# M4THYOU/TokenDagger

Measured on AMD Instinct MI355X. Metric: GB/s raw text tokenized (Llama-4 vocab, 1024 MB corpus), higher is better.
Workload: dtype u8

## Files before the change

### tokendagger_amd/csrc/td_kernels.hip

```cpp
#include <hip/hip_runtime.h>
#include <stdlib.h>

#include "td_kernels.h"

namespace td {

#ifdef TD_ABLATE
#define TD_STOP(n) (a.stop_after == (n))
#else
#define TD_STOP(n) false
#endif

struct LdsSrc {
    const uint8_t* txt;
    const uint32_t* docw;
    int64_t lo, hi;
    __device__ __forceinline__ uint32_t byte(int64_t i) const { return txt[i]; }
    __device__ __forceinline__ bool doc(int64_t i) const { return (docw[i >> 5] >> (i & 31)) & 1u; }
};
struct GlobSrc {
    const uint8_t* text;
    const uint32_t* docbits;
    int64_t lo, hi;
    __device__ __forceinline__ uint32_t byte(int64_t i) const { return text[i]; }
// ... 582 lines not shown
static_assert(SLAB_MIDS >= FZ_NPC + 8, "a slab holds the slots of the fullest tile the fused loop takes");
constexpr int FZ_R_BYTES = ((FZ_R_SPLIT_END > FZ_R_TOK_END ? FZ_R_SPLIT_END : FZ_R_TOK_END) + 15) & ~15;
constexpr int PD_KIND = 0;
constexpr int PD_TILE = 1, PD_NP = 2, PD_N0 = 3, PD_COUNT = 4, PD_NMISS = 5, PD_FDD = 6, PD_EXT0 = 7;
constexpr int PD_WORDS = 8;
static_assert(SLAB_MAX_MISSES == 2 * K_MISS_LISTED_MAX, "slab layout");
#ifndef TD_LB_MAX_POLLS
#define TD_LB_MAX_POLLS 2
#endif
#ifndef TD_LB_DRAIN_POLLS
#define TD_LB_DRAIN_POLLS 64
#endif
#ifndef TD_LB_MAX_ROUNDS
#define TD_LB_MAX_ROUNDS 4
#endif
#ifndef TD_FUSED_MIN_WAVES
#define TD_FUSED_MIN_WAVES 7
#endif

#ifndef TD_DIRECT_MIN_WAVES
#define TD_DIRECT_MIN_WAVES 6
#endif
static_assert(TD_FUSED_MIN_WAVES < 7 || FZ_R_BYTES <= 11072, "seven workgroups per CU: 22 752 B of LDS each, of which s_R may have 11 072");
template <uint32_t PV, bool FUSED, bool DIRECT>
__global__ __launch_bounds__(K_THREADS, !FUSED ? TD_SPLIT_MIN_WAVES : DIRECT ? TD_DIRECT_MIN_WAVES : TD_FUSED_MIN_WAVES) void td_split_tiles(const EncodeArgs a_kern) {
    static_assert(FUSED || !DIRECT, "direct placement is part of the fused tile loop");
    __shared__ __attribute__((aligned(16))) uint8_t s_txt[K_WIN];
    __shared__ __attribute__((aligned(16))) uint8_t s_R[FZ_R_BYTES];
    uint32_t* const s_cm = reinterpret_cast<uint32_t*>(s_R);
    uint16_t* const s_heads = reinterpret_cast<uint16_t*>(s_R + FZ_R_HEADS);
    uint16_t* const s_cold = reinterpret_cast<uint16_t*>(s_R + FZ_R_COLD);
    __shared__ uint32_t s_start[K_WIN / 32 + 3];
    __shared__ uint32_t s_doc[K_WIN / 32 + 2];
    __shared__ uint8_t s_lut[128];
    __shared__ uint8_t s_fcls[16];
    __shared__ uint32_t s_nh, s_cur, s_ncold, s_nonascii;
    __shared__ int s_last;
    __shared__ int s_cross;
    __shared__ uint32_t s_defer;
    __shared__ int s_next[2];

    const int tid = threadIdx.x;
#ifdef TD_FUSED_TIMING
    unsigned long long tt[16] = {0, 0, 0, 0, 0, 0, 0, 0, 0, 0, 0, 0, 0, 0, 0, 0}, t_last = __builtin_readcyclecounter(), t_total0 = t_last, n_tiles_done = 0;
#define FZ_TICK(i) { const unsigned long long t_now = __builtin_readcyclecounter(); tt[i] += t_now - t_last; t_last = t_now; FZ_FRESH }
#else
#define FZ_TICK(i) FZ_FRESH
#endif
#ifndef TD_ARGS_IN_REGISTERS
    (void)a_kern;
    FreshArgs a{kernarg_args()};
    FreshTables T{(const __attribute__((address_space(4))) Tables*)a->Tp};
#define FZ_FRESH { a.refresh(); T.refresh(); }
#else
    const KeptArgs a{&a_kern};
    const Tables T_kept = uniform_tables(a->Tp);
    const KeptTables T{&T_kept};
#define FZ_FRESH
#endif
    for (int q = tid; q < 128; q += K_THREADS) s_lut[q] = (uint8_t)feature_of_class(T->ascii_cls[q]);
    if (tid < 16) s_fcls[tid] = (uint8_t)feature_of_class((uint32_t)tid);
    if (tid == 0) s_nonascii = 0;
    if (tid < 2) s_doc[K_WIN / 32 + tid] = 0;
    static_assert(K_WIN / 32 + 2 == CM_STRIDE, "the document bits cover the words the stored masks have");
    __shared__ __attribute__((aligned(16))) uint32_t s_kmask[FUSED ? (P12_MAXLEN + 1) * 4 : 4];
    __shared__ uint32_t s_wave[8];
    __shared__ uint32_t s_hflags[2], s_nrec[2], s_ncoldp;
    __shared__ uint32_t s_rec[2][K_MISS_LISTED_MAX];
    __shared__ unsigned long long s_pend[48];
    __shared__ uint32_t s_npend;
// ... 25 lines not shown
        if (tid < (int)(P12_MAXLEN + 1) * 4) {
            const int len = tid >> 2, w = tid & 3, nb = len - 4 * w;
            s_kmask[tid] = w == 3 || nb <= 0 ? 0u : nb >= 4 ? 0xFFFFFFFFu : (1u << (8 * nb)) - 1u;
        }
        if (tid == 0) { s_nflagl = 0; s_npend = 0; s_brk = 0; }
        if (DIRECT && tid < SLAB_RING * PD_WORDS) (&s_pd[0][0])[tid] = 0;
        if (tid < 2) s_stat[tid] = 0;
    }
    __syncthreads();

#ifndef TD_FUSED_NPRE
#define TD_FUSED_NPRE 0
#endif
    constexpr int NPF = (K_WIN / 16 + K_THREADS - 1) / K_THREADS;
    constexpr int NPRE = FUSED ? TD_FUSED_NPRE : NPF;
    uint4 pf[NPF];
    const int64_t nwords = (a->n + 31) >> 5;
    auto interior = [&](int64_t w0) { return a->text_aligned && w0 >= 0 && w0 + K_WIN <= a->n; };
    uint32_t pfd0 = 0, pfd1 = 0, pffd0 = 0xFFFFFFFFu, pffd1 = 0xFFFFFFFFu;
#ifdef TD_TEXT_L2_PREFETCH
    uint32_t pft = 0;
#endif
    static_assert(K_WIN / 32 <= 2 * K_THREADS, "two prefetched document words per lane cover the window");
    auto load_window = [&](int64_t w0) {
        {
            const int64_t gw0 = (w0 >> 5) + tid, gw1 = gw0 + K_THREADS;
            pfd0 = (gw0 >= 0 && gw0 < nwords) ? a->docbits[gw0] : 0u;
            pfd1 = (tid < K_WIN / 32 - K_THREADS && gw1 >= 0 && gw1 < nwords) ? a->docbits[gw1] : 0u;
            if (FUSED) {
                const int64_t t4 = (w0 + K_HL) / K_TILE;
                pffd0 = t4 < a->n_tiles ? a->tile_first_doc[t4] : 0xFFFFFFFFu;
                pffd1 = t4 + 1 < a->n_tiles ? a->tile_first_doc[t4 + 1] : 0xFFFFFFFFu;
            }
        }
        if (!interior(w0)) return;
#ifdef TD_TEXT_L2_PREFETCH
        if (FUSED && NPRE == 0 && tid < (K_WIN + 63) / 64) pft = *reinterpret_cast<const volatile uint8_t*>(a->text + w0 + 64 * tid);
#endif
        const uint4* src16 = reinterpret_cast<const uint4*>(a->text + w0);
#pragma unroll
        for (int q = 0; q < NPRE; ++q)
            if (q < NPF - 1 || tid < K_WIN / 16 - (NPF - 1) * K_THREADS) pf[q] = nt_load16(src16 + q * K_THREADS + tid);
    };
#pragma unroll
    for (int q = 0; q < NPF; ++q) pf[q] = make_uint4(0, 0, 0, 0);
    int first_tile = (int)blockIdx.x;
    if constexpr (DIRECT) {
        if (tid == 0) s_next[0] = (int)atomicAdd(a->tile_draw, 1u);
        __syncthreads();
        first_tile = __builtin_amdgcn_readfirstlane(s_next[0]);
        __syncthreads();
    }
    if (first_tile < a->n_stiles) load_window((int64_t)first_tile * KS_TILE - K_HL);
    const int tid_outer = tid;
#ifndef TD_FUSED_STATIC_TILES
    constexpr bool DRAW = FUSED;
#else
    constexpr bool DRAW = false;
#endif
    int next_tile = 0, par = 0;
    int ring = 0;
    if (DRAW && !DIRECT && tid == 0) s_next[0] = (int)(blockIdx.x + gridDim.x);
    for (int tile = first_tile;; tile = DRAW ? next_tile : tile + (int)gridDim.x) {
        const bool have = tile < a->n_stiles;
        if (!have) {
            bool pending = false;
            if constexpr (DIRECT)
                for (int r = 0; r < SLAB_RING; ++r) pending = pending || s_pd[r][PD_KIND] != 0u;
            if (!pending) break;
        }
        int tid_opaque = tid_outer;
        asm volatile("" : "+v"(tid_opaque));
        const int tid = tid_opaque, lane = tid & 63;
        const int64_t tile_g0 = (int64_t)tile * KS_TILE;
        const int64_t wg0 = tile_g0 - K_HL;
        const int tile_hi = K_HL + (int)((a->n - tile_g0 < KS_TILE) ? (a->n - tile_g0) : KS_TILE);
// ... 9 lines not shown
        const uint32_t* const pslab = a->slab + ((size_t)blockIdx.x * SLAB_RING + ring) * SLAB_WORDS;
        if (DIRECT && pkind) {
            B = (int)s_pd[ring][PD_TILE];
            pnp = s_pd[ring][PD_NP]; pn0 = s_pd[ring][PD_N0]; pcount = s_pd[ring][PD_COUNT]; pnm = s_pd[ring][PD_NMISS]; pext0 = s_pd[ring][PD_EXT0];
            const uint32_t nv4 = (pnp + 3u) >> 2;
#pragma unroll
            for (int q = 0; q < 3; ++q) {
                xs[q] = make_uint4(0, 0, 0, 0);
                if ((uint32_t)tid + 256u * q < nv4) xs[q] = reinterpret_cast<const uint4*>(pslab)[tid + 256 * q];
            }
            const uint32_t pfdd = s_pd[ring][PD_FDD];
            pdm = (int64_t)pfdd + tid;
            pdpos = a->n;
            if (pkind == 1u && pfdd != 0xFFFFFFFFu && pdm < a->n_docs) { pdpos = a->doc_offsets[pdm]; pdsl = a->doc_slot[pdm]; }
            const int idx0 = B - 1 - tid;
            stw = (pkind == 1u && idx0 >= 0) ? __hip_atomic_load(&a->tile_state[idx0], __ATOMIC_RELAXED, __HIP_MEMORY_SCOPE_AGENT) : (TS_PREFIX << 62);
        }
        if (have) {
#ifdef TD_TEXT_L2_PREFETCH
        if (FUSED) asm volatile("" :: "v"(pft));
#endif

        uint32_t hib = 0;
        if (interior(wg0)) {
#pragma unroll
            for (int q = NPRE; q < NPF; ++q)
                if (q < NPF - 1 || tid < K_WIN / 16 - (NPF - 1) * K_THREADS) pf[q] = nt_load16(reinterpret_cast<const uint4*>(a->text + wg0) + q * K_THREADS + tid);
#pragma unroll
            for (int q = 0; q < NPF; ++q)
                if (q < NPF - 1 || tid < K_WIN / 16 - (NPF - 1) * K_THREADS) {
                    reinterpret_cast<uint4*>(s_txt)[q * K_THREADS + tid] = pf[q];
                    hib |= pf[q].x | pf[q].y | pf[q].z | pf[q].w;
                }
        } else {
            hib = stage_window_edge(s_txt, a->text, a->n, wg0, tid, K_WIN / 16);
        }
#pragma unroll
        for (int q = 0; q < 2; ++q) {
            const int w = tid + q * K_THREADS;
            if (w < K_WIN / 32) {
                uint32_t dw = q ? pfd1 : pfd0;
                const int64_t g = wg0 + (int64_t)w * 32;
                if (g + 32 > a->n) dw |= (g >= a->n) ? 0xFFFFFFFFu : ~((1u << (int)(a->n - g)) - 1u);
                s_doc[w] = dw;
            }
        }
        if (DRAW && DIRECT && tid == 0) s_next[0] = (int)atomicAdd(a->tile_draw, 1u);
        if (!FUSED && tile + (int)gridDim.x < a->n_stiles) load_window(wg0 + (int64_t)gridDim.x * KS_TILE);
        for (int w = tid; w < K_WIN / 32 + 3; w += K_THREADS) s_start[w] = 0;
        if (tid == 0) { s_nh = 0; s_cur = 0; s_ncold = 0; s_last = -1; s_cross = -1; s_defer = 0; }
        if (__ballot((hib & 0x80808080u) != 0) && lane == 0) s_nonascii = 1;
        }
        auto lb_post = [&](unsigned long long w) {
            const uint32_t status = (uint32_t)(w >> 62);
            const uint64_t na = __ballot(status != (uint32_t)TS_AGG);
            const int first = na ? (int)td_ctz64(na) : 64;
            const uint32_t mysum = wave_incl_scan(lane < first ? (uint32_t)w : 0u, lane);
            if (lane == 63) { s_lbs[tid >> 6][0] = (uint32_t)first; s_lbs[tid >> 6][1] = mysum; }
            if (lane == first) { s_lbs[tid >> 6][2] = status; s_lbv[tid >> 6] = w & TS_VALUE_MASK; }
        };
        if (DIRECT && pkind == 1u) lb_post(stw);
        __syncthreads();
        if (DIRECT && pkind) {
            const uint32_t* const slab = pslab;
            const uint32_t* const meta = slab + SLAB_META;
            const int64_t pg0 = (int64_t)B * KS_TILE, pg1 = (pg0 + KS_TILE < a->n) ? pg0 + KS_TILE : a->n;
            long long base = -1;
            if (pkind == 1u) {
                long long acc = 0;
                int j = B - 1, polls = 0, rounds = 0;
                for (;;) {
                    uint32_t tstatus = (uint32_t)TS_AGG;
                    unsigned long long tval = 0;
                    int tdist = 0;
#pragma unroll
                    for (int w = 0; w < K_THREADS / 64; ++w) {
                        if (tstatus == (uint32_t)TS_AGG) {
                            acc += s_lbs[w][1];
                            const int f = (int)s_lbs[w][0];
                            if (f < 64) { tstatus = s_lbs[w][2]; tval = s_lbv[w]; tdist = w * 64 + f; }
                        }
                    }
                    if (tstatus == (uint32_t)TS_PREFIX) { base = acc + (long long)tval; break; }
                    if (tstatus == (uint32_t)TS_BROKEN) { base = -1; break; }
                    if (tstatus == (uint32_t)TS_NONE) {
                        if (++polls > (have ? TD_LB_MAX_POLLS : TD_LB_DRAIN_POLLS)) { base = -2; break; }
                        j -= tdist;
                        __builtin_amdgcn_s_sleep(8);
                    } else {
                        if (++rounds >= TD_LB_MAX_ROUNDS) { base = -2; break; }
                        j -= K_THREADS;
                    }
                    __syncthreads();
                    const int idx = j - tid;
                    lb_post(idx >= 0 ? __hip_atomic_load(&a->tile_state[idx], __ATOMIC_RELAXED, __HIP_MEMORY_SCOPE_AGENT) : (TS_PREFIX << 62));
                    __syncthreads();
                }
            }
            FZ_TICK(8)
            const int tB4 = B * (KS_TILE / K_TILE);
            const bool ptwo = tB4 + 1 < a->n_tiles;
            uint32_t* const st0 = a->stage + (size_t)tB4 * K_STAGE;
            auto shift_of = [&](uint32_t k, int& mine) { return fz_shift_of(meta, pnm, k, &mine); };
            if (pkind == 1u && base >= 0) {
                int32_t* const dst = a->out_tokens + base;
                const bool fits = base + (long long)pcount <= (long long)a->out_cap;
                if (fits && pnm == 0u) {
#pragma unroll
                    for (int q = 0; q < 3; ++q) {
                        const uint32_t v = (uint32_t)tid + 256u * q;
                        if (4u * v + 4u <= pnp) {
                            u32x4a4 o;
                            o.x = xs[q].x; o.y = xs[q].y; o.z = xs[q].z; o.w = xs[q].w;
                            TD_NT_STORE(o, reinterpret_cast<u32x4a4*>(dst + 4u * v));
                        } else if (4u * v < pnp) {
                            dst[4u * v] = (int32_t)xs[q].x;
                            if (4u * v + 1u < pnp) dst[4u * v + 1u] = (int32_t)xs[q].y;
                            if (4u * v + 2u < pnp) dst[4u * v + 2u] = (int32_t)xs[q].z;
                        }
// ... 46 lines not shown
                    fz_stage_with_misses(slab, st0, a->merge_out + (size_t)tB4 * K_STAGE, pnp, pn0, pnm);
                }
                if (pkind == 1u && tid == 0) {
                    uint32_t m0 = 0, m1 = 0;
                    for (uint32_t q = 0; q < pnm; ++q) { if (meta[SLAB_MAX_MISSES + q] >> 12) m1 = 1; else m0 = 1; }
                    a->tile_count[tB4] = pn0 | (m0 ? TILE_MISS_LISTED : 0u);
                    a->tile_extra[tB4] = pext0;
                    if (ptwo) {
                        a->tile_count[tB4 + 1] = (pnp - pn0) | (m1 ? TILE_MISS_LISTED : 0u);
                        a->tile_extra[tB4 + 1] = pcount - pnp - pext0;
                    }
                    if (base == -1) {
                        __hip_atomic_store(&a->tile_state[B], TS_BROKEN << 62, __ATOMIC_RELAXED, __HIP_MEMORY_SCOPE_AGENT);
                        s_brk = 1u;
                    } else {
                        s_stat[1] += 1u;
                    }
                }
            }
            if (tid == 0) s_pd[ring][PD_KIND] = 0;
            FZ_TICK(11)
        }
        if (!have) {
            __syncthreads();
            ring = __builtin_amdgcn_readfirstlane(ring + 1 == SLAB_RING ? 0 : ring + 1);
            continue;
        }
        {
        FZ_TICK(0)
        const bool tile_ascii = !s_nonascii;

        LdsSrc src;
        src.txt = s_txt;
        src.docw = s_doc;
        src.lo = (wg0 < 0) ? -wg0 : 0;
        src.hi = (a->n - wg0 < K_WIN) ? (a->n - wg0) : K_WIN;
        if (tid < 2 * CM_COUNT) s_cm[(tid >> 1) * CM_STRIDE + 2 * K_MWORDS + (tid & 1)] = 0;
        auto emit_masks = [&](int it, uint32_t flo, uint32_t fhi, uint32_t pf) {
            const uint64_t P = transpose8x8(((uint64_t)fhi << 32) | flo);
            const uint32_t plo = (uint32_t)P, phi = (uint32_t)(P >> 32);
            const uint32_t mU = plo & 0xFF, mW = (plo >> 8) & 0xFF, mX = (plo >> 16) & 0xFF, mS = plo >> 24;
            const uint32_t nraw = phi & 0xFF, mCR = (phi >> 8) & 0xFF, mSL = (phi >> 16) & 0xFF, mC = phi >> 24;
            const uint32_t mN = nraw & ~mX & ~mS, mA = nraw & mX;
            const uint32_t mD = reinterpret_cast<const uint8_t*>(s_doc)[it];
            const uint32_t mSY = sync_byte(mU, mW, mX, mS, mN, mCR, mSL, mC, mD, mA, pf, PV);
            static_assert(CM_U == 0 && CM_W == 1 && CM_X == 2 && CM_S == 3 && CM_NRAW == 4 && CM_CR == 5 && CM_TR == 6 &&
                          CM_C == 7 && CM_SYNC == 8, "stored mask order");
            uint8_t* o = reinterpret_cast<uint8_t*>(s_cm) + it;
            constexpr int MB = CM_STRIDE * 4;
            o[0 * MB] = (uint8_t)mU; o[1 * MB] = (uint8_t)mW; o[2 * MB] = (uint8_t)mX; o[3 * MB] = (uint8_t)mS;
            o[4 * MB] = (uint8_t)nraw; o[5 * MB] = (uint8_t)mCR; o[6 * MB] = (uint8_t)(mCR | mSL); o[7 * MB] = (uint8_t)mC;
            o[8 * MB] = (uint8_t)mSY;
        };
        constexpr int P1_ITEMS = K_WIN / 8;
        if (tile_ascii) {
            for (int it = tid; it < P1_ITEMS; it += K_THREADS) {
                const uint2 t8 = reinterpret_cast<const uint2*>(s_txt)[it];
                const uint32_t flo = (uint32_t)s_lut[t8.x & 0x7F] | ((uint32_t)s_lut[(t8.x >> 8) & 0x7F] << 8) |
                                     ((uint32_t)s_lut[(t8.x >> 16) & 0x7F] << 16) | ((uint32_t)s_lut[t8.x >> 24] << 24);
                const uint32_t fhi = (uint32_t)s_lut[t8.y & 0x7F] | ((uint32_t)s_lut[(t8.y >> 8) & 0x7F] << 8) |
                                     ((uint32_t)s_lut[(t8.y >> 16) & 0x7F] << 16) | ((uint32_t)s_lut[t8.y >> 24] << 24);
                uint32_t pf = __shfl_up(fhi >> 24, 1);
                if (lane == 0) pf = it > 0 ? (uint32_t)s_lut[s_txt[it * 8 - 1]] : 0u;
                emit_masks(it, flo, fhi, pf);
            }
        } else {
        constexpr int P1_WAVES = K_THREADS / 64, P1_PER_WAVE = (P1_ITEMS / P1_WAVES) & ~63;
        static_assert(P1_ITEMS - P1_WAVES * P1_PER_WAVE <= 64, "the items left over are one more pass of the last wavefront");
        uint32_t carry_st = 0x100u, carry_pf = 0;
        const int n_pass = P1_PER_WAVE / 64 + ((tid >> 6) == P1_WAVES - 1 ? 1 : 0);
        const uint8_t* const t_ascii = T->ascii_cls;
        const uint16_t* const t_u1 = T->ucls1;
        const uint8_t* const t_u2 = T->ucls2;
        for (int q = 0; q < n_pass; ++q) {
            const int it = (tid >> 6) * P1_PER_WAVE + q * 64 + lane;
            if (it >= P1_ITEMS) break;
            const uint2 t8 = reinterpret_cast<const uint2*>(s_txt)[it];
            uint32_t flo, fhi;
            uint32_t st_out = 0;
// ... 100 lines not shown
                carry_st = (uint32_t)__builtin_amdgcn_readlane((int)st_out, 63);
                if (lead_conts) {
                    const bool known = !(st_in & 0x100u);
                    const int claim = (int)(st_in >> 9);
                    for (int k = 0; k < lead_conts; ++k) {
                        const uint32_t f = (known && k < claim) ? ((st_in & 0xFFu) | FB_C) : feature_at_v(t_ascii, t_u1, t_u2, s_txt, s_doc, (int)src.lo, (int)src.hi, it * 8 + k);
                        if (k < 4) flo |= f << (8 * k); else fhi |= f << (8 * (k - 4));
                    }
                }
            }
            uint32_t pf = __shfl_up(fhi >> 24, 1);
            if (lane == 0 && q > 0) pf = carry_pf;
            carry_pf = (uint32_t)__builtin_amdgcn_readlane((int)(fhi >> 24), 63);
            if (lane == 0 && q == 0) {
                pf = 0;
                if (it > 0) {
                    const uint32_t pb = s_txt[it * 8 - 1];
                    pf = (pb < 0x80) ? (uint32_t)s_lut[pb] : feature_at_v(t_ascii, t_u1, t_u2, s_txt, s_doc, (int)src.lo, (int)src.hi, it * 8 - 1);
                }
            }
            emit_masks(it, flo, fhi, pf);
        }
        }
        __syncthreads();
        FZ_TICK(1)
        if (tid == 0) s_nonascii = 0;
        if (TD_STOP(12)) continue;

        {
            constexpr bool FAST = !(PV & (PV_GPT2 | PV_LEADING_CONTRACTION | PV_PLAIN_LETTERS | PV_WS_EOS_FIRST));
            auto load_view64 = [&](BitWin& v, int j) {
                uint64_t s[CM_COUNT];
#pragma unroll
                for (int k = 0; k < CM_COUNT; ++k) s[k] = ((uint64_t)s_cm[k * CM_STRIDE + j + 1] << 32) | s_cm[k * CM_STRIDE + j];
                cm_expand(v, s, ((uint64_t)s_doc[j + 1] << 32) | s_doc[j]);
            };
            auto load_view32 = [&](BitWin32& v, int j, uint32_t sh) {
                uint32_t s[CM_COUNT];
#pragma unroll
                for (int k = 0; k < CM_COUNT; ++k) s[k] = __funnelshift_r(s_cm[k * CM_STRIDE + j], s_cm[k * CM_STRIDE + j + 1], sh);
                cm_expand(v, s, __funnelshift_r(s_doc[j], s_doc[j + 1], sh));
            };
            auto defer = [&](int64_t g) {
                if (FUSED) s_defer = 1;
                const uint32_t q = atomicAdd(a->slow_count, 1u);
                if (q < a->slow_cap) a->slow_list[q] = g;
                else raise(a, TD_E_SCRATCH, g);
// ... 29 lines not shown
                    un = (uint32_t)split_unresolved_heads(wv, PV, &extra) & sy;
                    extra &= (uint64_t)sy << 3;
                    extra &= room >= 64 ? ~0ull : room <= 0 ? 0ull : ((1ull << room) - 1ull);
                    st0 |= (uint32_t)extra;
                    extra_hi = (uint32_t)(extra >> 32);
                } else {
                    un = (uint32_t)split_unresolved_heads(wv, PV) & sy;
                }
                s_start[b0 >> 5] = st0;
                if (sy) atomicMax(&s_last, b0 + 31 - (int)__clz(sy));
                const uint32_t cnt = __popc(un);
                const uint32_t incl = wave_incl_scan(cnt, lane);
                uint32_t base = 0;
                if (lane == 63 && incl) base = atomicAdd(&s_nh, incl);
                base = (uint32_t)__builtin_amdgcn_readlane((int)base, 63);
                uint32_t idx = base + incl - cnt;
                while (un) {
                    const int bit = __ffs(un) - 1;
                    un &= un - 1u;
                    if (idx < (uint32_t)KS_HCAP) s_heads[idx] = (uint16_t)(b0 + bit); else mine |= 1u << bit;
                    ++idx;
                }
            }
            __syncthreads();
            FZ_TICK(2)
            if (extra_hi) atomicOr(&s_start[(b0 >> 5) + 1], extra_hi);
            if (TD_STOP(13)) continue;
            {
                const uint32_t nh = s_nh < (uint32_t)KS_HCAP ? s_nh : (uint32_t)KS_HCAP;
                int p = -1;
                if (tid == 0) {
                    static_assert(K_HL % 64 == 0 && K_HL >= 64, "left halo = whole mask words");
                    const uint32_t* const sync32 = s_cm + CM_SYNC * CM_STRIDE;
                    if (!(sync32[K_HL / 32] & 1u)) {
                        int sp = -1;
                        for (int w = K_HL / 64 - 1; w >= 0 && sp < 0; --w) {
                            uint64_t m = ((uint64_t)sync32[2 * w + 1] << 32) | sync32[2 * w];
                            if (w == 0) m &= ~0xFull;
                            if (m) sp = w * 64 + td_top64(m) - 1;
                        }
                        if (sp < 0) { a->tile_flag[tile] = 1; atomicAdd(a->far_count, 1u); if (FUSED) s_defer = 1; }
                        else p = sp;
                    }
                }
                if (tid == 1 && s_last >= 0) p = s_last;
                bool more = true;
                for (;;) {
                    const uint64_t nb = __ballot(p < 0);
                    if (nb && more) {
                        uint32_t base = 0;
                        if (lane == __ffsll((unsigned long long)nb) - 1) base = atomicAdd(&s_cur, (uint32_t)__popcll(nb));
                        base = (uint32_t)__builtin_amdgcn_readlane((int)base, __ffsll((unsigned long long)nb) - 1);
                        more = base + (uint32_t)__popcll(nb) < nh;
                        if (p < 0) {
                            const uint32_t idx = base + __builtin_amdgcn_mbcnt_hi((uint32_t)(nb >> 32), __builtin_amdgcn_mbcnt_lo((uint32_t)nb, 0u));
                            if (idx < nh) p = s_heads[idx];
                        }
                    }
                    if (!__ballot(p >= 0)) break;
                    if (p >= 0) {
                        BitWin32 v;
                        load_view32(v, p >> 5, (uint32_t)(p & 31));
                        const int avail = (K_LIM - p < 32) ? (K_LIM - p) : 32;
                        auto bytes = [&](int q) { return (uint32_t)s_txt[p + q]; };
                        const int r = FAST ? scan_piece_fast32(v, avail, bytes, PV) : scan_piece_p(WinP32(v, avail), bytes, PV);
                        if (r < 0) {
                            const uint32_t ci = atomicAdd(&s_ncold, 1u);
                            if (ci < (uint32_t)KS_CCAP) s_cold[ci] = (uint16_t)p; else walk(p);
                            p = -1;
                        } else {
                            const int e = p + r;
                            bool stop = true;
                            if (e >= tile_hi) crossed(e);
                            else {
                                stop = (r < 32) ? ((v.m[MK_SYNC] >> r) & 1u) : sync_at(e);
                                if (!stop && e >= K_HL) mark(e);
                            }
                            p = stop ? -1 : e;
                        }
                    }
                }
            }
            __syncthreads();
            {
                const uint32_t nc = s_ncold < (uint32_t)KS_CCAP ? s_ncold : (uint32_t)KS_CCAP;
                for (uint32_t i = tid; i < nc; i += K_THREADS) walk(s_cold[i]);
                while (mine) {
                    const int bit = __ffs(mine) - 1;
                    mine &= mine - 1u;
                    walk(b0 + bit);
                }
            }
        }
        __syncthreads();
        FZ_TICK(3)
        if (tid < KS_TILE / 32) {
            const int64_t g = tile_g0 + (int64_t)tid * 32;
            if (g < a->n) {
                uint32_t v = s_start[K_HL / 32 + tid];
                if (g + 32 > a->n) v &= (1u << (int)(a->n - g)) - 1u;
                TD_NT_STORE(v, &a->startbits[(tile_g0 >> 5) + tid]);
            }
        }
        if constexpr (DRAW) {
            if constexpr (!DIRECT) {
                next_tile = __builtin_amdgcn_readfirstlane(s_next[par]);
                if (tid == 0) s_next[par ^ 1] = (int)(2u * gridDim.x + atomicAdd(a->tile_draw, 1u));
                par = __builtin_amdgcn_readfirstlane(par ^ 1);
            } else {
                next_tile = __builtin_amdgcn_readfirstlane(s_next[0]);
            }
            if (next_tile < a->n_stiles) load_window((int64_t)next_tile * KS_TILE - K_HL);
        } else if (FUSED && tile + (int)gridDim.x < a->n_stiles) {
            load_window(wg0 + (int64_t)gridDim.x * KS_TILE);
        }
        }
        if constexpr (FUSED) {
            constexpr int NT4 = KS_TILE / K_TILE;
            static_assert(NT4 == 2 && KS_CHUNK == 32, "two token tiles, a 32-bit START word per lane");
            const int cross = s_cross;
            const bool tile_deferred = s_defer != 0 || cross < 0;
            uint16_t* const s_plist = reinterpret_cast<uint16_t*>(s_R + FZ_R_PLIST);
            uint16_t* const s_coldk = reinterpret_cast<uint16_t*>(s_R + FZ_R_COLDK);
            uint16_t* const s_pb = reinterpret_cast<uint16_t*>(s_R + FZ_R_PB);
            const int wv = tid >> 6;
            const int tile4 = tile * NT4;
            const bool two = K_HL + K_TILE < tile_hi;
            const int b0 = K_HL + tid * KS_CHUNK;
            const uint32_t smask0 = s_start[b0 >> 5];
            const uint32_t cnt = __popc(smask0);
            const uint32_t incl = wave_incl_scan(cnt, lane);
            if (lane == 63) s_wave[wv] = incl;
            if (tid == 0) { s_hflags[0] = 0; s_hflags[1] = 0; s_nrec[0] = 0; s_nrec[1] = 0; s_ncoldp = 0; }
            __syncthreads();
            const uint32_t w0s = s_wave[0], w1s = s_wave[1], w2s = s_wave[2], w3s = s_wave[3];
            const uint32_t np = w0s + w1s + w2s + w3s, n0 = w0s + w1s;
            const uint32_t pbase = (wv > 0 ? w0s : 0u) + (wv > 1 ? w1s : 0u) + (wv > 2 ? w2s : 0u) + incl - cnt;
            const bool cand = DIRECT && !s_brk;
            auto break_chain = [&]() {
                __hip_atomic_store(&a->tile_state[tile], TS_BROKEN << 62, __ATOMIC_RELAXED, __HIP_MEMORY_SCOPE_AGENT);
                s_brk = 1u;
            };
            if (tile_deferred || np > (uint32_t)FZ_NPC) {
                if (tid == 0) {
                    const uint32_t at = atomicAdd(a->deferred_count, two ? 2u : 1u);
                    a->deferred_list[at] = (uint32_t)tile4;
                    if (two) a->deferred_list[at + 1] = (uint32_t)tile4 + 1u;
                    if (DIRECT) break_chain();
                }
            } else {
                {
                    uint32_t k = pbase, m = smask0;
                    while (m) {
                        const int b = __ffs(m) - 1;
                        m &= m - 1;
                        s_plist[k++] = (uint16_t)(b0 + b);
                    }
                }
                s_pb[tid] = (uint16_t)pbase;
                if (tid == 0) s_plist[np] = (uint16_t)cross;
                const uint64_t fdd = fd0 != 0xFFFFFFFFu ? fd0 : fd1;
                if (cand && tid == 0) { s_pd[ring][PD_FDD] = (uint32_t)fdd; s_pd[ring][PD_TILE] = (uint32_t)tile; s_pd[ring][PD_NP] = np; s_pd[ring][PD_N0] = n0; }
                const int64_t dmine = (int64_t)fdd + tid;
                const int64_t dpos = (fdd != 0xFFFFFFFFu && dmine < a->n_docs) ? a->doc_offsets[dmine] : a->n;
                __syncthreads();
                FZ_TICK(4)
                uint32_t* const slab = a->slab + ((size_t)blockIdx.x * SLAB_RING + ring) * SLAB_WORDS;
                uint32_t* const dst0 = cand ? slab : a->stage + (size_t)tile4 * K_STAGE;
                uint32_t* const dst1 = cand ? slab : dst0 + K_STAGE - n0;
                auto note_miss = [&](uint32_t k, uint32_t res) {
                    const uint32_t h = k >= n0 ? 1u : 0u;
                    const uint32_t mi = atomicAdd(&s_nrec[h], 1u);
                    if (mi < (uint32_t)K_MISS_LISTED_MAX) s_rec[h][mi] = ((k - (h ? n0 : 0u)) << 19) | (res & 0x7FFFFu);
                };
                auto miss_marker = [&](int i, uint32_t len) { return TOK_MISS | ((uint32_t)((i - K_HL) & (K_TILE - 1)) << 7) | len; };
                typedef uint32_t u32x4 __attribute__((ext_vector_type(4)));
                typedef const u32x4 __attribute__((address_space(1)))* gslot_t;
                gslot_t const p12 = (gslot_t)(uintptr_t)T->piece12_slots;
                const uint32_t p12_mask = T->piece12_mask;
                const bool fastpath = a->use_fastpath != 0;
                for (uint32_t kb = tid; kb < np; kb += K_THREADS * FZ_PB) {
                    u32x4 sl[FZ_PB];
                    uint32_t kk0[FZ_PB], kk1[FZ_PB], kk2[FZ_PB], il[FZ_PB];
#pragma unroll
                    for (int q = 0; q < FZ_PB; ++q) {
                        const uint32_t k = kb + (uint32_t)q * K_THREADS;
                        const bool on = k < np;
                        const int i = on ? s_plist[k] : K_HL;
                        const uint32_t len = on ? (uint32_t)s_plist[k + 1] - (uint32_t)i : 0u;
                        const uint32_t* wp = reinterpret_cast<const uint32_t*>(s_txt) + (i >> 2);
                        const uint32_t sh = (i & 3) * 8;
                        const uint32_t w0 = wp[0], w1 = wp[1], w2 = wp[2], w3 = wp[3];
                        const uint4 km = reinterpret_cast<const uint4*>(s_kmask)[len < P12_MAXLEN ? len : P12_MAXLEN];
                        kk0[q] = __funnelshift_r(w0, w1, sh) & km.x;
                        kk1[q] = __funnelshift_r(w1, w2, sh) & km.y;
                        kk2[q] = __funnelshift_r(w2, w3, sh) & km.z;
                        il[q] = ((uint32_t)i << 16) | (len < 0xFFFFu ? len : 0xFFFFu);
                        if (on) sl[q] = p12[hash_piece12(kk0[q], kk1[q], kk2[q], len) & p12_mask];
                    }
#pragma unroll
                    for (int q = 0; q < FZ_PB; ++q) {
                        const uint32_t k = kb + (uint32_t)q * K_THREADS;
                        if (k < np) {
                            const int i = (int)(il[q] >> 16);
                            const uint32_t len = il[q] & 0xFFFFu;
                            const u32x4 e = sl[q];
                            if (len <= P12_MAXLEN && fastpath &&
                                (e.w == 0u || (e.x == kk0[q] && e.y == kk1[q] && e.z == kk2[q] && (e.w >> 24) == (0x80u | len)))) {
                                const bool miss = e.w == 0u;
                                const uint32_t res = miss ? miss_marker(i, len) : (e.w & 0x1FFFFFu);
                                if (miss) {
                                    if (len == 1) raise(a, TD_E_UNKNOWN_BYTE, wg0 + i);
                                    note_miss(k, res);
                                }
                                (k < n0 ? dst0 : dst1)[k] = res;
                            } else {
                                const uint32_t j = atomicAdd(&s_ncoldp, 1u);
                                if (j < (uint32_t)FZ_CCAP) s_coldk[j] = (uint16_t)k;
                            }
                        }
                    }
                }
                __syncthreads();
                FZ_TICK(5)
                const uint32_t ncold = s_ncoldp;
                const bool cold_overflow = ncold > (uint32_t)FZ_CCAP;
                if (!cold_overflow) {
                    for (uint32_t c = tid; c < ncold; c += K_THREADS) {
                        const uint32_t k = s_coldk[c];
                        const int i = s_plist[k];
                        const uint32_t len = (uint32_t)s_plist[k + 1] - (uint32_t)i;
                        const uint32_t h = k >= n0 ? 1u : 0u;
                        uint32_t res = probe_piece_cold<true>(a, T, s_txt, T->byte_id, &s_hflags[h], wg0, i, len);
                        if ((res & 0xC0000000u) == TOK_MISS) { res = miss_marker(i, len); note_miss(k, res); }
                        (h ? dst1 : dst0)[k] = res;
                    }
                }
                __syncthreads();
                FZ_TICK(6)
                const bool resolved = cand && !cold_overflow && !(s_hflags[0] | s_hflags[1]) && s_nrec[0] <= (uint32_t)K_MISS_LISTED_MAX &&
                                      s_nrec[1] <= (uint32_t)K_MISS_LISTED_MAX;
                if (cold_overflow) {
                    if (tid == 0) {
                        const uint32_t at = atomicAdd(a->deferred_count, two ? 2u : 1u);
                        a->deferred_list[at] = (uint32_t)tile4;
                        if (two) a->deferred_list[at + 1] = (uint32_t)tile4 + 1u;
                        if (DIRECT) break_chain();
                    }
                } else if (resolved) {
                    FZ_TICK(12)
                    if (tid < 64) {
                        const uint32_t nr0 = s_nrec[0], nr1 = s_nrec[1], nm = nr0 + nr1;
                        uint32_t ext0 = 0, ext1 = 0;
                        if (nm) {
                            static_assert(2 * SLAB_MAX_MISSES * 4 * MG_UNIT * 4 <= FZ_R_COLDK, "keys + ids of the merged pieces fit the (dead) piece list");
                            uint32_t rec = 0, hh = 0;
                            if ((uint32_t)lane < nm) {
                                hh = (uint32_t)lane >= nr0 ? 1u : 0u;
                                rec = s_rec[hh][(uint32_t)lane - (hh ? nr0 : 0u)];
                            }
                            const uint32_t nt = fz_merge_piece(a->Tp, a->text, a->n, reinterpret_cast<uint32_t*>(s_R), slab, rec, hh, n0, tile_g0, a->err, a->err_pos);
                            const uint32_t e0 = wave_incl_scan((nt && !hh) ? nt - 1u : 0u, lane), e1 = wave_incl_scan((nt && hh) ? nt - 1u : 0u, lane);
                            ext0 = (uint32_t)__builtin_amdgcn_readlane((int)e0, 63);
                            ext1 = (uint32_t)__builtin_amdgcn_readlane((int)e1, 63);
                        }
                        FZ_TICK(13)
                        if (tid == 0) {
                            const uint32_t count = s_pd[ring][PD_NP] + ext0 + ext1;
                            s_pd[ring][PD_KIND] = 1u; s_pd[ring][PD_COUNT] = count; s_pd[ring][PD_NMISS] = nm; s_pd[ring][PD_EXT0] = ext0;
                            __hip_atomic_store(&a->tile_state[s_pd[ring][PD_TILE]], (TS_AGG << 62) | (unsigned long long)count, __ATOMIC_RELAXED, __HIP_MEMORY_SCOPE_AGENT);
                        }
                    }
                    FZ_TICK(7)
                    {
                        const int64_t tile_end_g = wg0 + tile_hi;
                        auto slot_of = [&](int64_t p) {
                            const int lp = (int)(p - tile_g0);
                            const uint32_t k = (uint32_t)s_pb[lp >> 5] + __popc(s_start[K_HL / 32 + (lp >> 5)] & ((1u << (lp & 31)) - 1u));
                            return k >= n0 ? k - n0 : k;
                        };
                        if (dpos < tile_end_g) {
                            a->doc_slot[dmine] = slot_of(dpos);
                            for (int64_t d = dmine + K_THREADS; d < a->n_docs; d += K_THREADS) {
                                const int64_t p = a->doc_offsets[d];
                                if (p >= tile_end_g) break;
                                a->doc_slot[d] = slot_of(p);
                            }
                        }
                    }
                    FZ_TICK(9)
                } else {
                if (DIRECT && tid == 0) {
                    break_chain();
                    if (cand) { s_pd[ring][PD_KIND] = 2u; s_pd[ring][PD_NMISS] = 0; }
                }
                if (tid < 64) {
#pragma unroll
                    for (uint32_t h = 0; h < 2; ++h) {
                        const uint32_t nr = s_nrec[h], np0 = s_npend;
                        const bool listed = nr && nr <= (uint32_t)K_MISS_LISTED_MAX;
                        if (listed && (uint32_t)tid < nr) s_pend[np0 + tid] = ((unsigned long long)((uint32_t)tile4 + h) << 32) | s_rec[h][tid];
                        const uint32_t np1 = listed ? np0 + nr : np0;
                        wave_sync_lds();
                        if (np1 > 48u - (uint32_t)K_MISS_LISTED_MAX) {
                            append_pending(np1);
                            wave_sync_lds();
                            if (tid == 0) s_npend = 0;
                        } else if (tid == 0) {
                            s_npend = np1;
                        }
                        wave_sync_lds();
                    }
                    if (tid == 0) {
#pragma unroll
                        for (uint32_t h = 0; h < 2; ++h) {
                            if (h == 1 && !two) break;
                            uint32_t fl = s_hflags[h];
                            const uint32_t nr = s_nrec[h];
                            if (nr > (uint32_t)K_MISS_LISTED_MAX) {
                                fl |= TILE_HAS_MISS;
                                uint32_t nf = s_nflagl;
                                s_flagl[nf++] = (uint32_t)tile4 + h;
                                if (nf == 32u) {
                                    const uint32_t at = atomicAdd(a->flagged_count, 32u);
                                    for (uint32_t q = 0; q < 32u; ++q) a->flagged_list[at + q] = s_flagl[q];
                                    nf = 0;
                                }
                                s_nflagl = nf;
                            } else if (nr) {
                                fl |= TILE_MISS_LISTED;
                            }
                            a->tile_count[tile4 + h] = (h ? np - n0 : n0) | fl;
                        }
                    }
                }
                FZ_TICK(7)
                {
                    const int64_t tile_end_g = wg0 + tile_hi;
                    auto slot_of = [&](int64_t p) {
                        const int lp = (int)(p - tile_g0);
                        const uint32_t k = (uint32_t)s_pb[lp >> 5] + __popc(s_start[K_HL / 32 + (lp >> 5)] & ((1u << (lp & 31)) - 1u));
                        return k >= n0 ? k - n0 : k;
                    };
                    if (dpos < tile_end_g) {
                        a->doc_slot[dmine] = slot_of(dpos);
                        for (int64_t d = dmine + K_THREADS; d < a->n_docs; d += K_THREADS) {
                            const int64_t p = a->doc_offsets[d];
                            if (p >= tile_end_g) break;
                            a->doc_slot[d] = slot_of(p);
                        }
                    }
                }
                FZ_TICK(9)
                }
            }
        }
        __syncthreads();
        ring = __builtin_amdgcn_readfirstlane(ring + 1 == SLAB_RING ? 0 : ring + 1);
        FZ_TICK(10)
#ifdef TD_FUSED_TIMING
        ++n_tiles_done;
#endif
    }
#ifdef TD_FUSED_TIMING
    if (FUSED && tid == 0 && (blockIdx.x % 211) == 0)
        printf("fused wg %d: %llu tiles, total %llu cycles | stage %llu masks %llu rules %llu heads %llu | list %llu probe %llu cold %llu bookkeeping %llu lookback %llu docs %llu tail %llu place %llu | t12 %llu t13 %llu\n",
               (int)blockIdx.x, n_tiles_done, (unsigned long long)(__builtin_readcyclecounter() - t_total0), tt[0], tt[1], tt[2], tt[3], tt[4], tt[5], tt[6], tt[7],
               tt[8], tt[9], tt[10], tt[11], tt[12], tt[13]);
#endif
    if constexpr (FUSED) {
        if (DIRECT && tid == 0 && s_stat[0]) atomicAdd(a->direct_tiles, s_stat[0]);
        if (DIRECT && tid == 0 && s_stat[1]) atomicAdd(a->direct_tiles + 1, s_stat[1]);
        if (tid < 64) append_pending(s_npend);
        if (tid == 0 && s_nflagl) {
            const uint32_t nf = s_nflagl, at = atomicAdd(a->flagged_count, nf);
            for (uint32_t q = 0; q < nf; ++q) a->flagged_list[at + q] = s_flagl[q];
        }
    }
}

struct WaveMaskP {
    const Tables& T;
    const uint8_t* text;
    const uint32_t* docbits;
    int64_t n, g;
    int o, lim;
    int lane;
    __device__ __forceinline__ uint32_t cf_at(int64_t pos) const {
        if (pos >= n) return F_DOC;
        GlobSrc src;
        src.text = text; src.docbits = docbits; src.lo = 0; src.hi = n;
// ... 3582 lines not shown
```

Before: 494.5.

## Rotate serial duties across wavefronts per tile to balance barrier waits

Introduces a duty roster that gives single-lane and single-wave duties (head seeding, bookkeeping, draw, zeroing, cold lookups, doc slots, the tail of the text staging) to different wavefronts, rotating by tile index. The aim is to stop wavefront 0 from always carrying the serial work so the other waves are not idle at each workgroup barrier. It also turns the document-word loads into unconditional clamped loads and adds barrier-wait timing instrumentation. The risk is extra index arithmetic and possible divergence in the lane remapping.

```diff
diff --git a/tokendagger_amd/csrc/td_kernels.hip b/tokendagger_amd/csrc/td_kernels.hip
--- a/tokendagger_amd/csrc/td_kernels.hip
+++ b/tokendagger_amd/csrc/td_kernels.hip
@@ -628,6 +628,29 @@
 #define TD_DIRECT_MIN_WAVES 6
 #endif
 static_assert(TD_FUSED_MIN_WAVES < 7 || FZ_R_BYTES <= 11072, "seven workgroups per CU: 22 752 B of LDS each, of which s_R may have 11 072");
+
+#ifndef TD_ROSTER
+#define TD_ROSTER 3
+#endif
+constexpr bool RS_STATIC = (TD_ROSTER & 1) != 0, RS_TURN = (TD_ROSTER & 2) != 0;
+constexpr int RS_STAGE = 2, RS_MASK = 0, RS_HEAD_LEFT = 1, RS_HEAD_LAST = 2, RS_WALK = 3, RS_DRAW = 0, RS_LOOKUP = 2, RS_COLD = 1,
+              RS_BOOK = 2, RS_DOCS = 3;
+static_assert(((RS_LOOKUP + 3) & 3) == RS_COLD, "the lookup loop's short wavefront owns the cold lookups");
+static_assert(RS_HEAD_LEFT != RS_MASK && RS_HEAD_LAST != RS_MASK && RS_HEAD_LEFT != RS_HEAD_LAST && RS_BOOK != RS_DOCS && RS_WALK != RS_HEAD_LAST &&
+              RS_COLD != RS_BOOK, "neighbouring duties have different owners");
+__device__ __forceinline__ int duty_owner(int duty, int tile) {
+    return ((RS_STATIC ? duty : 0) + (RS_TURN ? tile : 0)) & 3;
+}
+__device__ __forceinline__ int duty_lane(int tid, int duty, int tile) {
+    if constexpr (!RS_STATIC && !RS_TURN) return tid;
+    return (tid - 64 * duty_owner(duty, tile)) & (K_THREADS - 1);
+}
+__device__ __forceinline__ bool duty_wave(int tid, int duty, int tile) {
+    if constexpr (!RS_STATIC && !RS_TURN) return tid < 64;
+    return (tid >> 6) == duty_owner(duty, tile);
+}
+static_assert(K_THREADS == 256, "four wavefronts take turns");
+
 template <uint32_t PV, bool FUSED, bool DIRECT>
 __global__ __launch_bounds__(K_THREADS, !FUSED ? TD_SPLIT_MIN_WAVES : DIRECT ? TD_DIRECT_MIN_WAVES : TD_FUSED_MIN_WAVES) void td_split_tiles(const EncodeArgs a_kern) {
     static_assert(FUSED || !DIRECT, "direct placement is part of the fused tile loop");
@@ -650,8 +673,11 @@
 #ifdef TD_FUSED_TIMING
     unsigned long long tt[16] = {0, 0, 0, 0, 0, 0, 0, 0, 0, 0, 0, 0, 0, 0, 0, 0}, t_last = __builtin_readcyclecounter(), t_total0 = t_last, n_tiles_done = 0;
 #define FZ_TICK(i) { const unsigned long long t_now = __builtin_readcyclecounter(); tt[i] += t_now - t_last; t_last = t_now; FZ_FRESH }
+    unsigned long long tb[16] = {0, 0, 0, 0, 0, 0, 0, 0, 0, 0, 0, 0, 0, 0, 0, 0};
+#define FZ_SYNC(i) { const unsigned long long t_in = __builtin_readcyclecounter(); __syncthreads(); tb[i] += __builtin_readcyclecounter() - t_in; }
 #else
 #define FZ_TICK(i) FZ_FRESH
+#define FZ_SYNC(i) __syncthreads()
 #endif
 #ifndef TD_ARGS_IN_REGISTERS
     (void)a_kern;
@@ -723,11 +749,20 @@
     uint32_t pft = 0;
 #endif
     static_assert(K_WIN / 32 <= 2 * K_THREADS, "two prefetched document words per lane cover the window");
-    auto load_window = [&](int64_t w0) {
+    auto load_window = [&](int64_t w0, int wtile) {
+        const int rs = duty_lane(tid, RS_STAGE, wtile);
+        (void)rs;
         {
             const int64_t gw0 = (w0 >> 5) + tid, gw1 = gw0 + K_THREADS;
-            pfd0 = (gw0 >= 0 && gw0 < nwords) ? a->docbits[gw0] : 0u;
-            pfd1 = (tid < K_WIN / 32 - K_THREADS && gw1 >= 0 && gw1 < nwords) ? a->docbits[gw1] : 0u;
+            const bool in0 = gw0 >= 0 && gw0 < nwords, in1 = tid < K_WIN / 32 - K_THREADS && gw1 >= 0 && gw1 < nwords;
+            if constexpr (RS_STATIC || RS_TURN) {
+                const uint32_t d0 = a->docbits[in0 ? gw0 : 0], d1 = a->docbits[in1 ? gw1 : 0];
+                pfd0 = in0 ? d0 : 0u;
+                pfd1 = in1 ? d1 : 0u;
+            } else {
+                pfd0 = in0 ? a->docbits[gw0] : 0u;
+                pfd1 = in1 ? a->docbits[gw1] : 0u;
+            }
             if (FUSED) {
                 const int64_t t4 = (w0 + K_HL) / K_TILE;
                 pffd0 = t4 < a->n_tiles ? a->tile_first_doc[t4] : 0xFFFFFFFFu;
@@ -741,7 +776,7 @@
         const uint4* src16 = reinterpret_cast<const uint4*>(a->text + w0);
 #pragma unroll
         for (int q = 0; q < NPRE; ++q)
-            if (q < NPF - 1 || tid < K_WIN / 16 - (NPF - 1) * K_THREADS) pf[q] = nt_load16(src16 + q * K_THREADS + tid);
+            if (q < NPF - 1 || rs < K_WIN / 16 - (NPF - 1) * K_THREADS) pf[q] = nt_load16(src16 + q * K_THREADS + (q < NPF - 1 ? tid : rs));
     };
 #pragma unroll
     for (int q = 0; q < NPF; ++q) pf[q] = make_uint4(0, 0, 0, 0);
@@ -752,7 +787,7 @@
         first_tile = __builtin_amdgcn_readfirstlane(s_next[0]);
         __syncthreads();
     }
-    if (first_tile < a->n_stiles) load_window((int64_t)first_tile * KS_TILE - K_HL);
+    if (first_tile < a->n_stiles) load_window((int64_t)first_tile * KS_TILE - K_HL, first_tile);
     const int tid_outer = tid;
 #ifndef TD_FUSED_STATIC_TILES
     constexpr bool DRAW = FUSED;
@@ -808,14 +843,16 @@
 #endif
 
         uint32_t hib = 0;
+        const int rs = duty_lane(tid, RS_STAGE, tile);
         if (interior(wg0)) {
 #pragma unroll
             for (int q = NPRE; q < NPF; ++q)
-                if (q < NPF - 1 || tid < K_WIN / 16 - (NPF - 1) * K_THREADS) pf[q] = nt_load16(reinterpret_cast<const uint4*>(a->text + wg0) + q * K_THREADS + tid);
+                if (q < NPF - 1 || rs < K_WIN / 16 - (NPF - 1) * K_THREADS)
+                    pf[q] = nt_load16(reinterpret_cast<const uint4*>(a->text + wg0) + q * K_THREADS + (q < NPF - 1 ? tid : rs));
 #pragma unroll
             for (int q = 0; q < NPF; ++q)
-                if (q < NPF - 1 || tid < K_WIN / 16 - (NPF - 1) * K_THREADS) {
-                    reinterpret_cast<uint4*>(s_txt)[q * K_THREADS + tid] = pf[q];
+                if (q < NPF - 1 || rs < K_WIN / 16 - (NPF - 1) * K_THREADS) {
+                    reinterpret_cast<uint4*>(s_txt)[q * K_THREADS + (q < NPF - 1 ? tid : rs)] = pf[q];
                     hib |= pf[q].x | pf[q].y | pf[q].z | pf[q].w;
                 }
         } else {
@@ -832,9 +869,9 @@
             }
         }
         if (DRAW && DIRECT && tid == 0) s_next[0] = (int)atomicAdd(a->tile_draw, 1u);
-        if (!FUSED && tile + (int)gridDim.x < a->n_stiles) load_window(wg0 + (int64_t)gridDim.x * KS_TILE);
-        for (int w = tid; w < K_WIN / 32 + 3; w += K_THREADS) s_start[w] = 0;
-        if (tid == 0) { s_nh = 0; s_cur = 0; s_ncold = 0; s_last = -1; s_cross = -1; s_defer = 0; }
+        if (!FUSED && tile + (int)gridDim.x < a->n_stiles) load_window(wg0 + (int64_t)gridDim.x * KS_TILE, tile + (int)gridDim.x);
+        for (int w = rs; w < K_WIN / 32 + 3; w += K_THREADS) s_start[w] = 0;
+        if (rs == (RS_STATIC ? 64 : 0)) { s_nh = 0; s_cur = 0; s_ncold = 0; s_last = -1; s_cross = -1; s_defer = 0; }
         if (__ballot((hib & 0x80808080u) != 0) && lane == 0) s_nonascii = 1;
         }
         auto lb_post = [&](unsigned long long w) {
@@ -846,7 +883,7 @@
             if (lane == first) { s_lbs[tid >> 6][2] = status; s_lbv[tid >> 6] = w & TS_VALUE_MASK; }
         };
         if (DIRECT && pkind == 1u) lb_post(stw);
-        __syncthreads();
+        FZ_SYNC(0);
         if (DIRECT && pkind) {
             const uint32_t* const slab = pslab;
             const uint32_t* const meta = slab + SLAB_META;
@@ -877,10 +914,10 @@
                         if (++rounds >= TD_LB_MAX_ROUNDS) { base = -2; break; }
                         j -= K_THREADS;
                     }
-                    __syncthreads();
+                    FZ_SYNC(8);
                     const int idx = j - tid;
                     lb_post(idx >= 0 ? __hip_atomic_load(&a->tile_state[idx], __ATOMIC_RELAXED, __HIP_MEMORY_SCOPE_AGENT) : (TS_PREFIX << 62));
-                    __syncthreads();
+                    FZ_SYNC(8);
                 }
             }
             FZ_TICK(8)
@@ -973,7 +1010,7 @@
             FZ_TICK(11)
         }
         if (!have) {
-            __syncthreads();
+            FZ_SYNC(0);
             ring = __builtin_amdgcn_readfirstlane(ring + 1 == SLAB_RING ? 0 : ring + 1);
             continue;
         }
@@ -986,7 +1023,11 @@
         src.docw = s_doc;
         src.lo = (wg0 < 0) ? -wg0 : 0;
         src.hi = (a->n - wg0 < K_WIN) ? (a->n - wg0) : K_WIN;
-        if (tid < 2 * CM_COUNT) s_cm[(tid >> 1) * CM_STRIDE + 2 * K_MWORDS + (tid & 1)] = 0;
+        const int rm = duty_lane(tid, RS_MASK, tile);
+        {
+            const int rz = RS_STATIC ? (rm + 128) & (K_THREADS - 1) : rm;
+            if (rz < 2 * CM_COUNT) s_cm[(rz >> 1) * CM_STRIDE + 2 * K_MWORDS + (rz & 1)] = 0;
+        }
         auto emit_masks = [&](int it, uint32_t flo, uint32_t fhi, uint32_t pf) {
             const uint64_t P = transpose8x8(((uint64_t)fhi << 32) | flo);
             const uint32_t plo = (uint32_t)P, phi = (uint32_t)(P >> 32);
@@ -1005,7 +1046,7 @@
         };
         constexpr int P1_ITEMS = K_WIN / 8;
         if (tile_ascii) {
-            for (int it = tid; it < P1_ITEMS; it += K_THREADS) {
+            for (int it = rm; it < P1_ITEMS; it += K_THREADS) {
                 const uint2 t8 = reinterpret_cast<const uint2*>(s_txt)[it];
                 const uint32_t flo = (uint32_t)s_lut[t8.x & 0x7F] | ((uint32_t)s_lut[(t8.x >> 8) & 0x7F] << 8) |
                                      ((uint32_t)s_lut[(t8.x >> 16) & 0x7F] << 16) | ((uint32_t)s_lut[t8.x >> 24] << 24);
@@ -1152,7 +1193,7 @@
             emit_masks(it, flo, fhi, pf);
         }
         }
-        __syncthreads();
+        FZ_SYNC(1);
         FZ_TICK(1)
         if (tid == 0) s_nonascii = 0;
         if (TD_STOP(12)) continue;
@@ -1228,14 +1269,16 @@
                     ++idx;
                 }
             }
-            __syncthreads();
+            FZ_SYNC(2);
             FZ_TICK(2)
             if (extra_hi) atomicOr(&s_start[(b0 >> 5) + 1], extra_hi);
             if (TD_STOP(13)) continue;
             {
                 const uint32_t nh = s_nh < (uint32_t)KS_HCAP ? s_nh : (uint32_t)KS_HCAP;
                 int p = -1;
-                if (tid == 0) {
+                const int rh = duty_lane(tid, RS_HEAD_LEFT, tile);
+                constexpr int RH_LAST = RS_STATIC ? 64 * ((RS_HEAD_LAST - RS_HEAD_LEFT) & 3) : 1;
+                if (rh == 0) {
                     static_assert(K_HL % 64 == 0 && K_HL >= 64, "left halo = whole mask words");
                     const uint32_t* const sync32 = s_cm + CM_SYNC * CM_STRIDE;
                     if (!(sync32[K_HL / 32] & 1u)) {
@@ -1249,7 +1292,7 @@
                         else p = sp;
                     }
                 }
-                if (tid == 1 && s_last >= 0) p = s_last;
+                if (rh == RH_LAST && s_last >= 0) p = s_last;
                 bool more = true;
                 for (;;) {
                     const uint64_t nb = __ballot(p < 0);
@@ -1287,10 +1330,10 @@
                     }
                 }
             }
-            __syncthreads();
+            FZ_SYNC(14);
             {
                 const uint32_t nc = s_ncold < (uint32_t)KS_CCAP ? s_ncold : (uint32_t)KS_CCAP;
-                for (uint32_t i = tid; i < nc; i += K_THREADS) walk(s_cold[i]);
+                for (uint32_t i = (uint32_t)duty_lane(tid, RS_WALK, tile); i < nc; i += K_THREADS) walk(s_cold[i]);
                 while (mine) {
                     const int bit = __ffs(mine) - 1;
                     mine &= mine - 1u;
@@ -1298,7 +1341,7 @@
                 }
             }
         }
-        __syncthreads();
+        FZ_SYNC(3);
         FZ_TICK(3)
         if (tid < KS_TILE / 32) {
             const int64_t g = tile_g0 + (int64_t)tid * 32;
@@ -1311,14 +1354,14 @@
         if constexpr (DRAW) {
             if constexpr (!DIRECT) {
                 next_tile = __builtin_amdgcn_readfirstlane(s_next[par]);
-                if (tid == 0) s_next[par ^ 1] = (int)(2u * gridDim.x + atomicAdd(a->tile_draw, 1u));
+                if (duty_lane(tid, RS_DRAW, tile) == 0) s_next[par ^ 1] = (int)(2u * gridDim.x + atomicAdd(a->tile_draw, 1u));
                 par = __builtin_amdgcn_readfirstlane(par ^ 1);
             } else {
                 next_tile = __builtin_amdgcn_readfirstlane(s_next[0]);
             }
-            if (next_tile < a->n_stiles) load_window((int64_t)next_tile * KS_TILE - K_HL);
+            if (next_tile < a->n_stiles) load_window((int64_t)next_tile * KS_TILE - K_HL, next_tile);
         } else if (FUSED && tile + (int)gridDim.x < a->n_stiles) {
-            load_window(wg0 + (int64_t)gridDim.x * KS_TILE);
+            load_window(wg0 + (int64_t)gridDim.x * KS_TILE, tile + (int)gridDim.x);
         }
         }
         if constexpr (FUSED) {
@@ -1337,8 +1380,9 @@
             const uint32_t cnt = __popc(smask0);
             const uint32_t incl = wave_incl_scan(cnt, lane);
             if (lane == 63) s_wave[wv] = incl;
-            if (tid == 0) { s_hflags[0] = 0; s_hflags[1] = 0; s_nrec[0] = 0; s_nrec[1] = 0; s_ncoldp = 0; }
-            __syncthreads();
+            const int rd = duty_lane(tid, RS_DRAW, tile);
+            if (rd == (RS_STATIC ? 64 : 0)) { s_hflags[0] = 0; s_hflags[1] = 0; s_nrec[0] = 0; s_nrec[1] = 0; s_ncoldp = 0; }
+            FZ_SYNC(4);
             const uint32_t w0s = s_wave[0], w1s = s_wave[1], w2s = s_wave[2], w3s = s_wave[3];
             const uint32_t np = w0s + w1s + w2s + w3s, n0 = w0s + w1s;
             const uint32_t pbase = (wv > 0 ? w0s : 0u) + (wv > 1 ? w1s : 0u) + (wv > 2 ? w2s : 0u) + incl - cnt;
@@ -1364,12 +1408,12 @@
                     }
                 }
                 s_pb[tid] = (uint16_t)pbase;
-                if (tid == 0) s_plist[np] = (uint16_t)cross;
+                if (rd == (RS_STATIC ? 128 : 0)) s_plist[np] = (uint16_t)cross;
                 const uint64_t fdd = fd0 != 0xFFFFFFFFu ? fd0 : fd1;
                 if (cand && tid == 0) { s_pd[ring][PD_FDD] = (uint32_t)fdd; s_pd[ring][PD_TILE] = (uint32_t)tile; s_pd[ring][PD_NP] = np; s_pd[ring][PD_N0] = n0; }
-                const int64_t dmine = (int64_t)fdd + tid;
+                const int64_t dmine = (int64_t)fdd + duty_lane(tid, RS_DOCS, tile);
                 const int64_t dpos = (fdd != 0xFFFFFFFFu && dmine < a->n_docs) ? a->doc_offsets[dmine] : a->n;
-                __syncthreads();
+                FZ_SYNC(4);
                 FZ_TICK(4)
                 uint32_t* const slab = a->slab + ((size_t)blockIdx.x * SLAB_RING + ring) * SLAB_WORDS;
                 uint32_t* const dst0 = cand ? slab : a->stage + (size_t)tile4 * K_STAGE;
@@ -1385,7 +1429,7 @@
                 gslot_t const p12 = (gslot_t)(uintptr_t)T->piece12_slots;
                 const uint32_t p12_mask = T->piece12_mask;
                 const bool fastpath = a->use_fastpath != 0;
-                for (uint32_t kb = tid; kb < np; kb += K_THREADS * FZ_PB) {
+                for (uint32_t kb = (uint32_t)duty_lane(tid, RS_LOOKUP, tile); kb < np; kb += K_THREADS * FZ_PB) {
                     u32x4 sl[FZ_PB];
                     uint32_t kk0[FZ_PB], kk1[FZ_PB], kk2[FZ_PB], il[FZ_PB];
 #pragma unroll
@@ -1427,12 +1471,12 @@
                         }
                     }
                 }
-                __syncthreads();
+                FZ_SYNC(5);
                 FZ_TICK(5)
                 const uint32_t ncold = s_ncoldp;
                 const bool cold_overflow = ncold > (uint32_t)FZ_CCAP;
                 if (!cold_overflow) {
-                    for (uint32_t c = tid; c < ncold; c += K_THREADS) {
+                    for (uint32_t c = (uint32_t)duty_lane(tid, RS_COLD, tile); c < ncold; c += K_THREADS) {
                         const uint32_t k = s_coldk[c];
                         const int i = s_plist[k];
                         const uint32_t len = (uint32_t)s_plist[k + 1] - (uint32_t)i;
@@ -1442,7 +1486,7 @@
                         (h ? dst1 : dst0)[k] = res;
                     }
                 }
-                __syncthreads();
+                FZ_SYNC(6);
                 FZ_TICK(6)
                 const bool resolved = cand && !cold_overflow && !(s_hflags[0] | s_hflags[1]) && s_nrec[0] <= (uint32_t)K_MISS_LISTED_MAX &&
                                       s_nrec[1] <= (uint32_t)K_MISS_LISTED_MAX;
@@ -1455,7 +1499,7 @@
                     }
                 } else if (resolved) {
                     FZ_TICK(12)
-                    if (tid < 64) {
+                    if (duty_wave(tid, RS_BOOK, tile)) {
                         const uint32_t nr0 = s_nrec[0], nr1 = s_nrec[1], nm = nr0 + nr1;
                         uint32_t ext0 = 0, ext1 = 0;
                         if (nm) {
@@ -1471,7 +1515,7 @@
                             ext1 = (uint32_t)__builtin_amdgcn_readlane((int)e1, 63);
                         }
                         FZ_TICK(13)
-                        if (tid == 0) {
+                        if (duty_lane(tid, RS_BOOK, tile) == 0) {
                             const uint32_t count = s_pd[ring][PD_NP] + ext0 + ext1;
                             s_pd[ring][PD_KIND] = 1u; s_pd[ring][PD_COUNT] = count; s_pd[ring][PD_NMISS] = nm; s_pd[ring][PD_EXT0] = ext0;
                             __hip_atomic_store(&a->tile_state[s_pd[ring][PD_TILE]], (TS_AGG << 62) | (unsigned long long)count, __ATOMIC_RELAXED, __HIP_MEMORY_SCOPE_AGENT);
@@ -1500,24 +1544,25 @@
                     break_chain();
                     if (cand) { s_pd[ring][PD_KIND] = 2u; s_pd[ring][PD_NMISS] = 0; }
                 }
-                if (tid < 64) {
+                if (duty_wave(tid, RS_BOOK, tile)) {
+                    const int bl = duty_lane(tid, RS_BOOK, tile);
 #pragma unroll
                     for (uint32_t h = 0; h < 2; ++h) {
                         const uint32_t nr = s_nrec[h], np0 = s_npend;
                         const bool listed = nr && nr <= (uint32_t)K_MISS_LISTED_MAX;
-                        if (listed && (uint32_t)tid < nr) s_pend[np0 + tid] = ((unsigned long long)((uint32_t)tile4 + h) << 32) | s_rec[h][tid];
+                        if (listed && (uint32_t)bl < nr) s_pend[np0 + bl] = ((unsigned long long)((uint32_t)tile4 + h) << 32) | s_rec[h][bl];
                         const uint32_t np1 = listed ? np0 + nr : np0;
                         wave_sync_lds();
                         if (np1 > 48u - (uint32_t)K_MISS_LISTED_MAX) {
                             append_pending(np1);
                             wave_sync_lds();
-                            if (tid == 0) s_npend = 0;
-                        } else if (tid == 0) {
+                            if (bl == 0) s_npend = 0;
+                        } else if (bl == 0) {
                             s_npend = np1;
                         }
                         wave_sync_lds();
                     }
-                    if (tid == 0) {
+                    if (bl == 0) {
 #pragma unroll
                         for (uint32_t h = 0; h < 2; ++h) {
                             if (h == 1 && !two) break;
@@ -1561,7 +1606,7 @@
                 }
             }
         }
-        __syncthreads();
+        FZ_SYNC(10);
         ring = __builtin_amdgcn_readfirstlane(ring + 1 == SLAB_RING ? 0 : ring + 1);
         FZ_TICK(10)
 #ifdef TD_FUSED_TIMING
@@ -1569,10 +1614,15 @@
 #endif
     }
 #ifdef TD_FUSED_TIMING
-    if (FUSED && tid == 0 && (blockIdx.x % 211) == 0)
-        printf("fused wg %d: %llu tiles, total %llu cycles | stage %llu masks %llu rules %llu heads %llu | list %llu probe %llu cold %llu bookkeeping %llu lookback %llu docs %llu tail %llu place %llu | t12 %llu t13 %llu\n",
-               (int)blockIdx.x, n_tiles_done, (unsigned long long)(__builtin_readcyclecounter() - t_total0), tt[0], tt[1], tt[2], tt[3], tt[4], tt[5], tt[6], tt[7],
-               tt[8], tt[9], tt[10], tt[11], tt[12], tt[13]);
+    if (FUSED && (tid & 63) == 0 && (blockIdx.x % 53) == 0) {
+        const uint32_t hw = __builtin_amdgcn_s_getreg(4 | (31 << 11)), xcc = __builtin_amdgcn_s_getreg(20 | (31 << 11));
+        unsigned long long tb_all = 0;
+        for (int q = 0; q < 16; ++q) tb_all += tb[q];
+        printf("fused wg %d wave %d simd %u cu %u xcc %u hw_id 0x%08x roster %d: %llu tiles, total %llu cycles, at barriers %llu | stage %llu masks %llu rules %llu heads %llu | list %llu probe %llu cold %llu bookkeeping %llu lookback %llu docs %llu tail %llu place %llu | t12 %llu t13 %llu | waits: stage %llu masks %llu rules %llu heads-b %llu heads %llu list %llu probe %llu cold %llu tail %llu\n",
+               (int)blockIdx.x, tid >> 6, (hw >> 4) & 3u, (hw >> 8) & 15u, xcc & 15u, hw, (int)TD_ROSTER, n_tiles_done,
+               (unsigned long long)(__builtin_readcyclecounter() - t_total0), tb_all, tt[0], tt[1], tt[2], tt[3], tt[4], tt[5], tt[6], tt[7],
+               tt[8], tt[9], tt[10], tt[11], tt[12], tt[13], tb[0], tb[1], tb[2], tb[14], tb[3], tb[4], tb[5], tb[6], tb[10]);
+    }
 #endif
     if constexpr (FUSED) {
         if (DIRECT && tid == 0 && s_stat[0]) atomicAdd(a->direct_tiles, s_stat[0]);
```

Result: no change. 492.6 (-0.4%).
